# avi22bhattacharya/ThinkDiff-mlre

Hardware: AMD Instinct MI355X
Metric: images/sec (1024², 28 steps) ThinkDiff-CLIP FLUX.1 at 1/2/4/8 MI355X (higher is better)
Workload: dtype bf16

## Files before the change

### thinkdiff-mlre_amd/csrc/attention_bf16.hip

```cpp
#include "attention_common.h"

template <bool Q8>
__device__ __forceinline__ void attn_store_item(const TdAttnParams& p, const f32x16_t (&o)[4], const float inv, bf16_t* Ob, const int Sq,
                                                const int head, const int q, const int h5) {
  if constexpr (Q8) {
    if (p.q8) {
      const int qr = min(q, Sq - 1);
      attn_store_rows_q8(o, inv, p.q8 + (size_t)qr * p.ldq8 + head * D, h5, p.q8_inv[qr], p.q8_amax + qr, q < Sq);
      return;
    }
  }
  attn_store_rows(o, inv, Ob + (size_t)min(q, Sq - 1) * p.ldo + head * D, h5, (p.ldo & 7) == 0 && !(p.variant & 0x200), q < Sq);
}

template <bool CAUSAL, int NWAVES, bool BIAS = false, bool VARLEN = false, bool PRE = false, bool RS = true, bool FIXED = false, bool KVSEG = false>
__global__ __launch_bounds__(NWAVES * 64, 2) void td_attn_fwd_d128_lean_kernel(const TdAttnParams p) {
#if defined(__HIP_DEVICE_COMPILE__)
  extern __shared__ __attribute__((aligned(16))) char smem[];

  const int tid = threadIdx.x;
  const int lane = tid & 63;
  const int wid = __builtin_amdgcn_readfirstlane(tid >> 6);
  const int h5 = lane >> 5;
  const int l31 = lane & 31;

  const int qblk = blockIdx.x;
  const int head = blockIdx.y;
  const int batch = blockIdx.z;
  const int kvhead = head / p.q_per_kv;
  const int q0 = qblk * (NWAVES * Q_WAVE) + wid * Q_WAVE;

  const bf16_t* Qb = p.Q + (size_t)batch * p.q_bstride;
  const bf16_t* Kb = p.K + (size_t)batch * p.kv_bstride;
  const bf16_t* Vb = p.V + (size_t)batch * p.kv_bstride;
  bf16_t* Ob = p.O + (size_t)batch * p.o_bstride;
  int Sq = p.Sq, Skv = p.Skv, c_off = p.causal_offset;
  if constexpr (VARLEN) {
    const int r0 = p.seg_starts[batch];
    Sq = Skv = p.seg_starts[batch + 1] - r0;
    if (qblk * (NWAVES * Q_WAVE) >= Sq) return;
    if constexpr (KVSEG) {
      const int k0 = max(p.kv_seg_row0[batch], 0);
      Skv = max(p.kv_seg_lens[batch], Sq);
      c_off = Skv - Sq;
      Qb += (size_t)r0 * p.ldq; Kb += (size_t)k0 * p.ldkv; Vb += (size_t)k0 * p.ldkv; Ob += (size_t)r0 * p.ldo;
    } else {
      Qb += (size_t)r0 * p.ldq; Kb += (size_t)r0 * p.ldkv; Vb += (size_t)r0 * p.ldkv; Ob += (size_t)r0 * p.ldo;
    }
  }

  const unsigned q_bytes = (unsigned)(((long long)(Sq - 1) * p.ldq + p.Hq * D) * 2);
  if constexpr (CAUSAL) {
    if (p.kv_lens) { Skv = p.kv_lens[batch]; c_off = Skv - p.Sq; }
  }
  const unsigned kv_bytes = (unsigned)(((long long)(Skv - 1) * p.ldkv + p.Hkv * D) * 2);
  __amdgpu_buffer_rsrc_t rsQ = __builtin_amdgcn_make_buffer_rsrc((void*)Qb, 0, q_bytes, 0x00020000);
  __amdgpu_buffer_rsrc_t rsK = __builtin_amdgcn_make_buffer_rsrc((void*)Kb, 0, kv_bytes, 0x00020000);
  __amdgpu_buffer_rsrc_t rsV = __builtin_amdgcn_make_buffer_rsrc((void*)Vb, 0, kv_bytes, 0x00020000);

  int nt = (Skv + KV_TILE - 1) / KV_TILE;
  if (CAUSAL) {
    const int last_q = min(Sq, (qblk + 1) * NWAVES * Q_WAVE) - 1 + c_off;
    nt = min(nt, last_q / KV_TILE + 1);
  }

  constexpr int GROUPS = KV_TILE / 4;
  constexpr int SG = (GROUPS + NWAVES - 1) / NWAVES;
  const int srow = lane >> 4;
  unsigned voffK[SG];
#pragma unroll
  for (int s = 0; s < SG; ++s) {
    const int g = wid + NWAVES * s;
    const int swz = (srow << 2) | (g & 3);
    const int chunk = (lane & 15) ^ swz;
    voffK[s] = (unsigned)(g * 4 + srow) * (unsigned)p.ldkv * 2u + (unsigned)(kvhead * D + chunk * 8) * 2u;
  }
  auto stage = [&](int slot, int t) {
    const unsigned tile_off = (unsigned)t * KV_TILE * (unsigned)p.ldkv * 2u;
#pragma unroll
    for (int s = 0; s < SG; ++s) {
      const int g = wid + NWAVES * s;
      if (GROUPS % NWAVES == 0 || g < GROUPS) {
        __builtin_amdgcn_raw_ptr_buffer_load_lds(rsK, (TD_LDS void*)(smem + slot * TILE_BYTES + g * 1024), 16, voffK[s] + tile_off, 0, 0, 0);
        __builtin_amdgcn_raw_ptr_buffer_load_lds(rsV, (TD_LDS void*)(smem + (2 + slot) * TILE_BYTES + g * 1024), 16, voffK[s] + tile_off, 0, 0, 0);
      }
    }
  };
  stage(0, 0);

  bf16x8_t qf[8];
  {
    const unsigned qoff = (unsigned)(q0 + l31) * (unsigned)p.ldq * 2u + (unsigned)(head * D + 8 * h5) * 2u;
#pragma unroll
    for (int ks = 0; ks < 8; ++ks) {
      u32x4_t v = __builtin_amdgcn_raw_buffer_load_b128(rsQ, qoff + ks * 32, 0, 0);
      qf[ks] = __builtin_bit_cast(bf16x8_t, v);
    }
  }

  const unsigned lds0 = (unsigned)(uintptr_t)(TD_LDS char*)smem;
  unsigned ka[8];
  {
    const unsigned ksw = ((lane & 3) << 2) | ((lane >> 2) & 3);
#pragma unroll
    for (int ks = 0; ks < 8; ++ks) ka[ks] = lds0 + l31 * 256 + (((2 * ks + h5) ^ ksw) << 4);
  }
  unsigned va[2][4];
  {
    const unsigned vq = (lane & 15) >> 2, vp = lane & 3;
    const unsigned vchunk = 2 * ((lane >> 4) & 1) + (vp >> 1);
#pragma unroll
    for (int jj = 0; jj < 2; ++jj) {
      const unsigned swz = (vq << 2) | ((2 * jj + h5) & 3);
#pragma unroll
      for (int db = 0; db < 4; ++db)
        va[jj][db] = lds0 + 2 * TILE_BYTES + (4 * h5 + vq + 8 * jj) * 256 + (((4 * db + vchunk) ^ swz) << 4) + 8 * (vp & 1);
    }
  }

  f32x16_t o[4];
#pragma unroll
// ... 36 lines not shown
            for (int r = 0; r < 4; ++r) st[kb][4 * g4 + r] += bv[r] * inv_scale;
          }
        }
    }
    const bool need_mask = (key0 + KV_TILE > Skv) || (CAUSAL && key0 + KV_TILE - 1 > q0 + c_off);
    if (need_mask) {
#pragma unroll
      for (int kb = 0; kb < 2; ++kb)
#pragma unroll
        for (int r = 0; r < 16; ++r) {
          const int key = key0 + kb * 32 + (r & 3) + 8 * (r >> 2) + 4 * h5;
          if ((key >= Skv) || (CAUSAL && key > q_pos)) st[kb][r] = -INFINITY;
        }
    }

    attn_tile_softmax_pv<PO, PRE, RS, FIXED>(st, o, lacc, m_run, qnegm, t == 0, c, va, h5);
  };
  {
    int t = 0;
    for (; t + 1 < nt; t += 2) {
      tile(t, std::integral_constant<unsigned, 0>{});
      tile(t + 1, std::integral_constant<unsigned, 1>{});
    }
    if (t < nt) tile(t, std::integral_constant<unsigned, 0>{});
  }

  const float inv = 1.0f / (RS ? lacc[0] : half_swap_sum(lacc[0]));
  attn_store_item<!CAUSAL && !BIAS && !VARLEN>(p, o, inv, Ob, Sq, head, q0 + l31, h5);
#endif
}



template <int NWAVES, bool XCD_REMAP, bool PRE = false, bool RS = true, bool FIXED = false>
__global__ __launch_bounds__(NWAVES * 64, 2) void td_attn_fwd_d128_streamk_kernel(const TdAttnParams p, char* __restrict__ ws,
                                                                                  const int n_qblk, const int nt) {
#if defined(__HIP_DEVICE_COMPILE__)
  extern __shared__ __attribute__((aligned(16))) char smem[];
  const int tid = threadIdx.x;
  const int lane = tid & 63;
  const int wid = __builtin_amdgcn_readfirstlane(tid >> 6);
  const int h5 = lane >> 5;
  const int l31 = lane & 31;
  TD_LDS unsigned* const ticket_lds = (TD_LDS unsigned*)(smem + 4 * TILE_BYTES);

  const int G = gridDim.x;
  long long it, it_end;
  const int r = attn_sk_range<XCD_REMAP>((long long)n_qblk * p.Hq * p.batch * nt, it, it_end);

  const int Skv = p.Skv;
  constexpr int GROUPS = KV_TILE / 4;
  constexpr int SG = (GROUPS + NWAVES - 1) / NWAVES;
  const int srow = lane >> 4;
  const float c = p.scale * 1.4426950408889634f;
  const float cc = PRE ? 1.0f : c;
  const bf16x8_t kone = {(short)(h5 == 0 ? 0x3F80 : 0), 0, 0, 0, 0, 0, 0, 0};

  const unsigned lds0 = (unsigned)(uintptr_t)(TD_LDS char*)smem;
  unsigned ka[8];
  {
    const unsigned ksw = ((lane & 3) << 2) | ((lane >> 2) & 3);
#pragma unroll
    for (int ks = 0; ks < 8; ++ks) ka[ks] = lds0 + l31 * 256 + (((2 * ks + h5) ^ ksw) << 4);
  }
  unsigned va[2][4];
  {
    const unsigned vq = (lane & 15) >> 2, vp = lane & 3;
    const unsigned vchunk = 2 * ((lane >> 4) & 1) + (vp >> 1);
#pragma unroll
    for (int jj = 0; jj < 2; ++jj) {
      const unsigned swz = (vq << 2) | ((2 * jj + h5) & 3);
#pragma unroll
      for (int db = 0; db < 4; ++db)
        va[jj][db] = lds0 + 2 * TILE_BYTES + (4 * h5 + vq + 8 * jj) * 256 + (((4 * db + vchunk) ^ swz) << 4) + 8 * (vp & 1);
    }
  }

  if ((p.variant & 0x100) && wid >= 4) __builtin_amdgcn_s_setprio(1);
  while (it < it_end) {
    const int item = (int)(it / nt);
    const int kb = (int)(it - (long long)item * nt);
    const int ke = (int)min((long long)nt, kb + (it_end - it));
    __builtin_assume(ke > kb);
    it += ke - kb;
    const int qblk = item % n_qblk;
    const int hb = item / n_qblk;
    const int head = hb % p.Hq, batch = hb / p.Hq;
    const int kvhead = head / p.q_per_kv;
    const int q0 = qblk * (NWAVES * Q_WAVE) + wid * Q_WAVE;

    const bf16_t* Qb = p.Q + (size_t)batch * p.q_bstride;
    const bf16_t* Kb = p.K + (size_t)batch * p.kv_bstride;
    const bf16_t* Vb = p.V + (size_t)batch * p.kv_bstride;
    const unsigned q_bytes = (unsigned)(((long long)(p.Sq - 1) * p.ldq + p.Hq * D) * 2);
    const unsigned kv_bytes = (unsigned)(((long long)(Skv - 1) * p.ldkv + p.Hkv * D) * 2);
    __amdgpu_buffer_rsrc_t rsQ = __builtin_amdgcn_make_buffer_rsrc((void*)Qb, 0, q_bytes, 0x00020000);
    __amdgpu_buffer_rsrc_t rsK = __builtin_amdgcn_make_buffer_rsrc((void*)Kb, 0, kv_bytes, 0x00020000);
    __amdgpu_buffer_rsrc_t rsV = __builtin_amdgcn_make_buffer_rsrc((void*)Vb, 0, kv_bytes, 0x00020000);

    unsigned voffK[SG];
#pragma unroll
    for (int s = 0; s < SG; ++s) {
      const int g = wid + NWAVES * s;
      const int swz = (srow << 2) | (g & 3);
      const int chunk = (lane & 15) ^ swz;
      voffK[s] = (unsigned)(g * 4 + srow) * (unsigned)p.ldkv * 2u + (unsigned)(kvhead * D + chunk * 8) * 2u;
    }
    auto stage = [&](int slot, int t) {
      const unsigned tile_off = (unsigned)t * KV_TILE * (unsigned)p.ldkv * 2u;
#pragma unroll
      for (int s = 0; s < SG; ++s) {
        const int g = wid + NWAVES * s;
        if (GROUPS % NWAVES == 0 || g < GROUPS) {
          __builtin_amdgcn_raw_ptr_buffer_load_lds(rsK, (TD_LDS void*)(smem + slot * TILE_BYTES + g * 1024), 16, voffK[s] + tile_off, 0, 0, 0);
          __builtin_amdgcn_raw_ptr_buffer_load_lds(rsV, (TD_LDS void*)(smem + (2 + slot) * TILE_BYTES + g * 1024), 16, voffK[s] + tile_off, 0, 0, 0);
        }
      }
    };
    __syncthreads();
    stage(0, kb);

    bf16x8_t qf[8];
    {
      const unsigned qoff = (unsigned)(q0 + l31) * (unsigned)p.ldq * 2u + (unsigned)(head * D + 8 * h5) * 2u;
#pragma unroll
      for (int ks = 0; ks < 8; ++ks) {
        u32x4_t v = __builtin_amdgcn_raw_buffer_load_b128(rsQ, qoff + ks * 32, 0, 0);
        qf[ks] = __builtin_bit_cast(bf16x8_t, v);
      }
    }

    f32x16_t o[4];
#pragma unroll
    for (int db = 0; db < 4; ++db)
#pragma unroll
      for (int rr = 0; rr < 16; ++rr) o[db][rr] = 0.f;
    f32x16_t lacc;
#pragma unroll
    for (int rr = 0; rr < 16; ++rr) lacc[rr] = 0.f;
    float m_run = 0.f;
    bf16x8_t qnegm = {0, 0, 0, 0, 0, 0, 0, 0};
    auto tile = [&](const int t, auto slot_tag) {
      constexpr unsigned SLOT = decltype(slot_tag)::value;
      constexpr unsigned PO = SLOT * TILE_BYTES;
      asm volatile("s_waitcnt vmcnt(0)" ::: "memory");
      __syncthreads();
      if (t + 1 < ke) stage(SLOT ^ 1, t + 1);

      f32x16_t st[2];
      attn_tile_scores<PO, FIXED>(st, qf, kone, qnegm, ka);

      const int key0 = t * KV_TILE;
      if (key0 + KV_TILE > Skv) {
// ... 83 lines not shown
  }
  if (p.Sq == 1 && p.causal && !p.bias && !p.seg_starts && (p.variant & 0xff) == 0 && (p.kv_lens || p.causal_offset == p.Skv - 1))
    return td_attn_decode_launch(p, stream);
  TdAttnParams q = p;
  q.q_per_kv = p.Hq / p.Hkv;
  constexpr int NW = 8;
  constexpr int lds = 4 * TILE_BYTES;
  int dev = 0;
  TD_CHECK_HIP(hipGetDevice(&dev));
  dim3 grid((p.Sq + NW * Q_WAVE - 1) / (NW * Q_WAVE), p.Hq, p.batch);
  if (p.bias) TD_CHECK_ARG(p.Skv % 4 == 0 && ((uintptr_t)p.bias) % 16 == 0 && p.batch == 1, "td_attention: bias needs Skv %% 4 == 0, 16-byte alignment, batch 1");
  if (p.kv_lens) TD_CHECK_ARG(p.causal && !p.bias, "td_attention: per-sequence kv lengths exist for the causal kernel only");
  if (p.q_prescaled) TD_CHECK_ARG(!p.causal && !p.bias && !p.kv_lens && !p.seg_starts, "td_attention: pre-scaled q is a form of the joint (unmasked) attention only");
  TD_CHECK_ARG(p.score_bound >= 0.f && p.score_bound <= 48.f && (p.score_bound == 0.f || p.q_prescaled), "td_attention: a score bound goes with pre-scaled q (joint attention) and lies in (0, 48] octaves (0 = none)");
  if (p.q8) TD_CHECK_ARG(!p.causal && !p.bias && !p.kv_lens && !p.seg_starts && p.batch == 1 && p.q8_inv && p.q8_amax && p.ldq8 % 8 == 0 && ((uintptr_t)p.q8) % 8 == 0,
                         "td_attention: the int8 output form is for the joint attention of one batch entry, with 8-byte aligned rows");
  if (p.seg_starts && p.kv_seg_row0) {
    if (int e = attn_launch<td_attn_fwd_d128_lean_kernel<true, NW, false, true, false, true, false, true>>(grid, NW * 64, lds, stream, dev, q)) return e;
    TD_CHECK_LAUNCH();
    return 0;
  }
  if (p.seg_starts) {
    TD_CHECK_ARG(!p.bias && !p.kv_lens && p.Sq == p.Skv && (!p.causal || p.causal_offset == 0),
                 "td_attention(varlen): full or causal (offset 0) attention inside each segment only (no bias or cache lengths)");
    if (int e = p.causal ? attn_launch<td_attn_fwd_d128_lean_kernel<true, NW, false, true>>(grid, NW * 64, lds, stream, dev, q)
                         : attn_launch<td_attn_fwd_d128_lean_kernel<false, NW, false, true>>(grid, NW * 64, lds, stream, dev, q)) return e;
    TD_CHECK_LAUNCH();
    return 0;
  }

  const int n_items = (int)(grid.x * grid.y * grid.z);
  const int cus = device_cus(dev);
  const int nt = (p.Skv + KV_TILE - 1) / KV_TILE;
  int e;
  if (!p.causal && !p.bias && !p.kv_lens && (p.variant & 0xff) != 1 && cus > 0 && n_items > cus && cus < SK_MAX_RANGES && (long long)n_items * nt < (1ll << 31)) {
    char* ws = (char*)p.sk_ws;
    if (!ws) {
      if (int rc = sk_pooled_workspace(dev, cus, stream, &ws)) return rc;
    }
    constexpr int lds_sk = lds + 16;
    const dim3 ranges(cus);
    const int n_qblk = (int)grid.x;
    if (p.q_prescaled && p.score_bound > 0.f) e = attn_launch<td_attn_fwd_d128_streamk_kernel<NW, true, true, true, true>>(ranges, NW * 64, lds_sk, stream, dev, q, ws, n_qblk, nt);
    else if (p.q_prescaled) e = attn_launch<td_attn_fwd_d128_streamk_kernel<NW, true, true>>(ranges, NW * 64, lds_sk, stream, dev, q, ws, n_qblk, nt);
    else if ((p.variant & 0xff) == 2) e = attn_launch<td_attn_fwd_d128_streamk_kernel<NW, false>>(ranges, NW * 64, lds_sk, stream, dev, q, ws, n_qblk, nt);
    else e = attn_launch<td_attn_fwd_d128_streamk_kernel<NW, true>>(ranges, NW * 64, lds_sk, stream, dev, q, ws, n_qblk, nt);
  } else if (p.bias) {
    e = p.causal ? attn_launch<td_attn_fwd_d128_lean_kernel<true, NW, true>>(grid, NW * 64, lds, stream, dev, q)
                 : attn_launch<td_attn_fwd_d128_lean_kernel<false, NW, true>>(grid, NW * 64, lds, stream, dev, q);
  } else if (p.q_prescaled && p.score_bound > 0.f) {
    e = attn_launch<td_attn_fwd_d128_lean_kernel<false, NW, false, false, true, true, true>>(grid, NW * 64, lds, stream, dev, q);
  } else if (p.q_prescaled) {
    e = attn_launch<td_attn_fwd_d128_lean_kernel<false, NW, false, false, true>>(grid, NW * 64, lds, stream, dev, q);
  } else {
    e = p.causal ? attn_launch<td_attn_fwd_d128_lean_kernel<true, NW>>(grid, NW * 64, lds, stream, dev, q)
                 : attn_launch<td_attn_fwd_d128_lean_kernel<false, NW>>(grid, NW * 64, lds, stream, dev, q);
  }
  if (e) return e;
  TD_CHECK_LAUNCH();
  return 0;
}

size_t td_attn_streamk_ws_bytes() {
  int dev = 0;
  if (hipGetDevice(&dev) != hipSuccess) return 0;
  const int cus = device_cus(dev);
  return cus > 0 && cus < SK_MAX_RANGES ? sk_ws_bytes(cus) : 0;
}
```

### thinkdiff-mlre_amd/csrc/attention_common.h

```cpp
#pragma once
#include <atomic>
#include <mutex>
#include <type_traits>
#include <vector>

#include "td_common.h"
#include "td_kernels.h"

namespace {

constexpr int D = 128;
constexpr int KV_TILE = 64;
constexpr int Q_WAVE = 32;
constexpr int TILE_BYTES = KV_TILE * D * 2;

__device__ __forceinline__ void half_swap(float x, float& lo, float& hi) {
  lo = x;
  hi = x;
  asm volatile("s_nop 1\n\tv_permlane32_swap_b32 %0, %1\n\ts_nop 1" : "+v"(lo), "+v"(hi));
}
__device__ __forceinline__ float max3(float a, float b, float c) {
  float r;
  asm("v_max3_f32 %0, %1, %2, %3" : "=v"(r) : "v"(a), "v"(b), "v"(c));
  return r;
// ... 154 lines not shown
        w[0] = pack_bf2(o[db][4 * g] * inv, o[db][4 * g + 1] * inv);
        w[1] = pack_bf2(o[db][4 * g + 2] * inv, o[db][4 * g + 3] * inv);
        if (live) *(u32x2_t*)(row_ptr + 4 * h5 + db * 32 + 8 * g) = w;
      }
  }
}

__device__ __forceinline__ void attn_store_rows_q8(const f32x16_t (&o)[4], const float inv, uint8_t* row_ptr, const int h5, const float qinv, unsigned* amax,
                                                   const bool live) {
  float am = 0.f;
#pragma unroll
  for (int db = 0; db < 4; ++db)
#pragma unroll
    for (int g = 0; g < 4; g += 2) {
      unsigned w[2];
#pragma unroll
      for (int h = 0; h < 2; ++h) {
        unsigned acc = 0;
#pragma unroll
        for (int b = 0; b < 4; ++b) {
          const float v = rbf(o[db][4 * (g + h) + b] * inv);
          am = fmaxf(am, fabsf(v));
          acc |= ((unsigned)__float2int_rn(fminf(fmaxf(v * qinv, -127.f), 127.f)) & 0xffu) << (8 * b);
        }
        w[h] = acc;
      }
      const auto r = __builtin_amdgcn_permlane32_swap(w[0], w[1], false, false);
      if (live) *(u32x2_t*)(row_ptr + db * 32 + 8 * (g + h5)) = u32x2_t{r[0], r[1]};
    }
  am = half_swap_max(am);
  if (live && h5 == 0) __hip_atomic_fetch_max(amax, as_u32(am), __ATOMIC_RELAXED, __HIP_MEMORY_SCOPE_AGENT);
}

constexpr int SK_SLOT_FLOATS = 8 * 64 * 68;
constexpr int SK_HEADER_BYTES = 4096;
constexpr int SK_MAX_RANGES = SK_HEADER_BYTES / 4 - 16;

template <bool XCD_REMAP>
__device__ __forceinline__ int attn_sk_range(const long long total, long long& it, long long& it_end) {
  const int G = gridDim.x;
  int r = blockIdx.x;
  if constexpr (XCD_REMAP) {
    const int q8 = G >> 3, r8 = G & 7, xcd = r & 7;
    r = (xcd < r8 ? xcd * (q8 + 1) : r8 * (q8 + 1) + (xcd - r8) * q8) + (r >> 3);
  }
  it = total * r / G;
  it_end = total * (r + 1) / G;
  return r;
}

__device__ __forceinline__ bool attn_sk_handoff(f32x16_t (&o_io)[4], const float m_run, float& l_run, const float cc, const int r, const int G,
                                                const bool tail, char* ws, TD_LDS unsigned* const ticket_lds, const int tid, const int wid) {
  const int lane = tid & 63;
  f32x16_t o[4] = {o_io[0], o_io[1], o_io[2], o_io[3]};
  unsigned* const cnt = (unsigned*)ws + 16;
  const int j = tail ? r : r + 1;
  const __amdgpu_buffer_rsrc_t rsS = __builtin_amdgcn_make_buffer_rsrc((void*)(ws + SK_HEADER_BYTES), 0, (unsigned)(2 * G) * SK_SLOT_FLOATS * 4u, 0x00020000);
  const unsigned lane_off = ((unsigned)wid * 17u * 64u + (unsigned)lane) * 16u;
  const unsigned mine = (unsigned)(tail ? j : G + j) * (SK_SLOT_FLOATS * 4u) + lane_off;
  const unsigned theirs = (unsigned)(tail ? G + j : j) * (SK_SLOT_FLOATS * 4u) + lane_off;
  auto ask = [&](bool draw) -> unsigned {
    __syncthreads();
    if (tid == 0)
      *ticket_lds = draw ? __hip_atomic_fetch_add(cnt + j, 1u, __ATOMIC_RELAXED, __HIP_MEMORY_SCOPE_AGENT)
                         : __hip_atomic_load(cnt + j, __ATOMIC_RELAXED, __HIP_MEMORY_SCOPE_AGENT);
    __syncthreads();
    return *ticket_lds;
  };
  bool other_ready = !tail && ask(false) == 1u;
  if (!other_ready) {
#pragma unroll
    for (int q4 = 0; q4 < 16; ++q4) {
      const u32x4_t v = {as_u32(o[q4 >> 2][4 * (q4 & 3)]), as_u32(o[q4 >> 2][4 * (q4 & 3) + 1]),
                         as_u32(o[q4 >> 2][4 * (q4 & 3) + 2]), as_u32(o[q4 >> 2][4 * (q4 & 3) + 3])};
      __builtin_amdgcn_raw_buffer_store_b128(v, rsS, mine + q4 * 1024u, 0, 16);
    }
    const u32x4_t ml = {as_u32(m_run), as_u32(l_run), 0u, 0u};
    __builtin_amdgcn_raw_buffer_store_b128(ml, rsS, mine + 16 * 1024u, 0, 16);
    asm volatile("s_waitcnt vmcnt(0)" ::: "memory");
    other_ready = ask(true) == 1u;
    if (!other_ready) return false;
  }
  if (tid == 0) __builtin_amdgcn_fence(__ATOMIC_ACQUIRE, "agent");
  asm volatile("s_waitcnt vmcnt(0)" ::: "memory");
  __syncthreads();
  const u32x4_t ml = __builtin_amdgcn_raw_buffer_load_b128(rsS, theirs + 16 * 1024u, 0, 0);
  const float m2 = as_f32(ml[0]), l2 = as_f32(ml[1]);
  const float mm = fmaxf(m_run, m2);
  const float a1 = __builtin_amdgcn_exp2f((m_run - mm) * cc), a2 = __builtin_amdgcn_exp2f((m2 - mm) * cc);
  auto comb = [&](float own, float other) {
    return tail ? __builtin_fmaf(other, a2, own * a1) : __builtin_fmaf(own, a1, other * a2);
  };
  l_run = comb(l_run, l2);
#pragma unroll
  for (int q4 = 0; q4 < 16; ++q4) {
    const u32x4_t v = __builtin_amdgcn_raw_buffer_load_b128(rsS, theirs + q4 * 1024u, 0, 0);
#pragma unroll
    for (int k4 = 0; k4 < 4; ++k4)
      o[q4 >> 2][4 * (q4 & 3) + k4] = comb(o[q4 >> 2][4 * (q4 & 3) + k4], as_f32(v[k4]));
  }
  if (tid == 0) __hip_atomic_store(cnt + j, 0u, __ATOMIC_RELAXED, __HIP_MEMORY_SCOPE_AGENT);
#pragma unroll
  for (int db = 0; db < 4; ++db) o_io[db] = o[db];
  return true;
}

template <auto KERNEL, typename... Args>
int attn_launch(const dim3 grid, const int threads, const int lds, hipStream_t stream, const int dev, Args... args) {
  static std::atomic<unsigned long long> done{0};
  if (!((done.load(std::memory_order_acquire) >> (dev & 63)) & 1ull)) {
    TD_CHECK_HIP(hipFuncSetAttribute((const void*)KERNEL, hipFuncAttributeMaxDynamicSharedMemorySize, lds));
    done.fetch_or(1ull << (dev & 63), std::memory_order_release);
  }
  hipLaunchKernelGGL(KERNEL, grid, dim3(threads), lds, stream, args...);
  return 0;
}

}
```

### thinkdiff-mlre_amd/csrc/capi.hip

```cpp
#include <cstdarg>
#include <cstdio>
#include <initializer_list>
#include "td_kernels.h"
#include "../../include/thinkdiff_hip.h"

static thread_local char g_err[512] = "";

void td_set_error(const char* fmt, ...) {
  va_list ap;
  va_start(ap, fmt);
  vsnprintf(g_err, sizeof(g_err), fmt, ap);
  va_end(ap);
}

extern "C" {

const char* td_last_error(void) { return g_err; }
int td_abi_version(void) { return 24; }

int td_linear_bf16(const void* x, int64_t ldx, const void* w, const void* bias, void* y, int64_t ldy,
                   int M, int N, int K, int act, const void* gate, const void* res, int64_t ldr,
                   void* stream) {
  TdGemmParams p;
  p.A = (const bf16_t*)x; p.lda = (int)ldx;
// ... 78 lines not shown
int td_linear_f32out_bf16(const void* x, int64_t ldx, const void* w, const void* bias, float* y, int64_t ldy,
                          int M, int N, int K, void* stream) {
  TdGemmParams p;
  p.A = (const bf16_t*)x; p.lda = (int)ldx; p.W = (const bf16_t*)w; p.bias = (const bf16_t*)bias;
  p.C = (bf16_t*)y; p.ldc = (int)ldy; p.M = M; p.N = N; p.K = K; p.out_f32 = 1; p.cfg = (N <= 64) ? 1 : (M <= 32 ? 2 : 0);
  return td_gemm_launch(p, (hipStream_t)stream);
}

static int g_attn_variant = 0;
int td_attention_set_variant(int variant) {
  const int prev = g_attn_variant;
  g_attn_variant = variant;
  return prev;
}

int td_attention_bf16(const void* q, int64_t ldq, int64_t q_bstride, const void* k, const void* v,
                      int64_t ldkv, int64_t kv_bstride, void* o, int64_t ldo, int64_t o_bstride,
                      int batch, int Sq, int Skv, int Hq, int Hkv, int head_dim, float scale,
                      int causal, void* stream) {
  TdAttnParams p;
  p.Q = (const bf16_t*)q; p.K = (const bf16_t*)k; p.V = (const bf16_t*)v; p.O = (bf16_t*)o;
  p.batch = batch; p.Sq = Sq; p.Skv = Skv; p.Hq = Hq; p.Hkv = Hkv; p.head_dim = head_dim;
  p.ldq = (int)ldq; p.ldkv = (int)ldkv; p.ldo = (int)ldo;
  p.q_bstride = q_bstride; p.kv_bstride = kv_bstride; p.o_bstride = o_bstride;
  p.scale = scale; p.causal = causal; p.causal_offset = Skv - Sq; p.variant = g_attn_variant & ~0x800;
  p.q_prescaled = (g_attn_variant & 0x800) && !causal ? 1 : 0;
  return td_attn_launch(p, (hipStream_t)stream);
}

int td_attention_joint_prescaled_bf16(const void* q, int64_t ldq, const void* k, const void* v, int64_t ldkv, void* o, int64_t ldo, int S, int H, float score_bound, void* stream) {
  TdAttnParams p;
  p.Q = (const bf16_t*)q; p.K = (const bf16_t*)k; p.V = (const bf16_t*)v; p.O = (bf16_t*)o;
  p.batch = 1; p.Sq = S; p.Skv = S; p.Hq = H; p.Hkv = H; p.head_dim = 128;
  p.ldq = (int)ldq; p.ldkv = (int)ldkv; p.ldo = (int)ldo; p.scale = 1.0f; p.causal = 0; p.causal_offset = 0; p.variant = g_attn_variant & 0xff;
  p.q_prescaled = 1; p.score_bound = score_bound;
  return td_attn_launch(p, (hipStream_t)stream);
}

size_t td_attention_fp8_workspace_bytes(int Sq, int Skv, int Hq) { return Sq > 0 && Skv > 0 && Hq > 0 ? td_attn_fp8_ws_bytes(Sq, Skv, Hq) : 0; }

int td_attention_fp8(const void* q, int64_t ldq, const void* k, const void* v, int64_t ldkv, void* o, int64_t ldo,
                     int Sq, int Skv, int Hq, float scale, void* workspace, void* stream) {
  TdAttnParams p;
  p.Q = (const bf16_t*)q; p.K = (const bf16_t*)k; p.V = (const bf16_t*)v; p.O = (bf16_t*)o;
  p.batch = 1; p.Sq = Sq; p.Skv = Skv; p.Hq = Hq; p.Hkv = Hq; p.head_dim = 128;
  p.ldq = (int)ldq; p.ldkv = (int)ldkv; p.ldo = (int)ldo; p.scale = scale; p.f8_ws = workspace; p.variant = ((g_attn_variant & 1) ? 0x1000 : 0) | ((g_attn_variant & 2) ? 0x2000 : 0) | (((g_attn_variant >> 4) & 7) << 16);
  return td_attn_fp8_launch(p, (hipStream_t)stream);
}

int td_attention_fp8_qk_rope(const void* qkv, int64_t ld, int q_col, int k_col, int v_col, void* o, int64_t ldo, int S, int H,
                             const float* cos, const float* sin, int split, const void* wqA, const void* wkA, const void* wqB, const void* wkB,
                             float eps, float scale, void* workspace, void* stream) {
  TD_CHECK_ARG(qkv && cos && sin && q_col >= 0 && k_col >= 0 && v_col >= 0 && (q_col | k_col | v_col) % 8 == 0, "td_attention_fp8_qk_rope: projection buffer, both tables, 16-byte aligned column offsets");
  TD_CHECK_ARG(S > 0 && H > 0 && (long long)(q_col > k_col ? (q_col > v_col ? q_col : v_col) : (k_col > v_col ? k_col : v_col)) + (long long)H * 128 <= ld,
               "td_attention_fp8_qk_rope: the q / k / v head blocks (H=%d x 128 columns from their offsets) do not fit a row of ld=%lld", H, (long long)ld);
  TdAttnParams p;
  p.Q = (const bf16_t*)qkv + q_col; p.K = (const bf16_t*)qkv + k_col; p.V = (const bf16_t*)qkv + v_col; p.O = (bf16_t*)o;
  p.batch = 1; p.Sq = S; p.Skv = S; p.Hq = H; p.Hkv = H; p.head_dim = 128;
  p.ldq = (int)ld; p.ldkv = (int)ld; p.ldo = (int)ldo; p.scale = scale; p.f8_ws = workspace; p.variant = ((g_attn_variant & 1) ? 0x1000 : 0) | ((g_attn_variant & 2) ? 0x2000 : 0);
  p.rope_cos = cos; p.rope_sin = sin; p.rope_split = split; p.rope_eps = eps;
  p.rope_wqA = (const bf16_t*)wqA; p.rope_wkA = (const bf16_t*)wkA; p.rope_wqB = (const bf16_t*)wqB; p.rope_wkB = (const bf16_t*)wkB;
  return td_attn_fp8_launch(p, (hipStream_t)stream);
}

int td_attention_varlen_bf16(const void* q, int64_t ldq, const void* k, const void* v, int64_t ldkv, void* o, int64_t ldo,
                             const int* seg_starts, int n_seg, int max_len, int Hq, int Hkv, float scale, void* stream) {
  TD_CHECK_ARG(seg_starts && n_seg > 0 && max_len > 0, "td_attention_varlen: empty segment list");
// ... 650 lines not shown
```

### thinkdiff-mlre_amd/csrc/flux_engine.hip

```cpp
#include <cmath>
#include <cstring>
#include <functional>

#include "flux_model.h"

namespace {

struct TraceScope {
  td_flux* f; hipStream_t s; bool on;
  TraceScope(td_flux* f_, hipStream_t s_, int cat, double flops) : f(f_), s(s_), on(f_->tracing) {
    if (!on) return;
    const size_t i = f->trace.size();
    if (2 * i + 1 >= f->ev_pool.size()) { on = false; return; }
    f->trace.push_back({cat, flops});
    (void)hipEventRecord(f->ev_pool[2 * i], s);
  }
  ~TraceScope() {
    if (on) (void)hipEventRecord(f->ev_pool[2 * (f->trace.size() - 1) + 1], s);
  }
};

int gemm_p(td_flux* f, hipStream_t s, TdGemmParams p) {
  p.no_tail = f->shared_chip;
  const int rows = p.M + p.g_M;
// ... 95 lines not shown
}

int norm_rows(td_flux* f, hipStream_t s, const TdNormParams& p) {
  TraceScope ts(f, s, TD_TRACE_NORM, 0.0);
  return td_norm_rows_launch(p, s);
}
int qk_rope(td_flux* f, hipStream_t s, const TdQkRopeParams& p) {
  TraceScope ts(f, s, TD_TRACE_QKROPE, 0.0);
  return td_qk_norm_rope_launch(p, s);
}
int attn(td_flux* f, hipStream_t s, const TdAttnParams& p, const TdQkRopeParams* rope = nullptr, const int* ref_in = nullptr, int* ref_out = nullptr) {
  TraceScope ts(f, s, TD_TRACE_ATTN, 4.0 * p.Sq * (double)p.Skv * p.Hq * 128.0);
  if (f->m->attn_mode == TD_ATTENTION_FP8) {
    TdAttnParams q = p;
    q.f8_ws = f->attn8_ws;
    q.variant = p.variant & 0x1000;
    q.ref_in = ref_in; q.ref_out = ref_out;
    if (rope) {
      const TdQkRopeParams& r = *rope;
      q.rope_cos = r.cos; q.rope_sin = r.sin; q.rope_split = r.split; q.rope_eps = r.eps; q.rope_q_premul = r.q_premul;
      q.rope_wqA = r.wqA; q.rope_wkA = r.wkA; q.rope_wqB = r.wqB; q.rope_wkB = r.wkB;
    }
    return td_attn_fp8_launch(q, s);
  }
  return td_attn_launch(p, s);
}

struct Switches {
  int attn_tune;
  bool attn8_no_fuse;
  bool attn8_no_href;
  bool attn_no_bound;
  static Switches read() {
    static const int tune = getenv("TD_ATTN_TUNE") ? (int)strtol(getenv("TD_ATTN_TUNE"), nullptr, 0) & ~0xff : 0;
    return {tune, getenv("TD_ATTN8_NO_FUSE") != nullptr, getenv("TD_ATTN8_NO_HREF") != nullptr, getenv("TD_ATTN_NO_BOUND") != nullptr};
  }
};

int alloc_workspace(td_flux* f) {
  const FluxModel* m = f->m;
  const TdFluxConfig* cfg = &m->cfg;
  const int64_t D = m->D, M = m->M;
  const int max_img_tokens = m->max_img, max_txt_tokens = m->max_txt + (m->num_mode > 0 ? 1 : 0);
  const int64_t S = (int64_t)max_img_tokens + max_txt_tokens;
  const int64_t n = m->max_steps;
  struct Req { void** p; int64_t bytes; };
  std::vector<Req> reqs = {
      {(void**)&f->h, S * D * 2}, {(void**)&f->xn, S * D * 2}, {(void**)&f->qkv, S * 3 * D * 2},
      {(void**)&f->attn, S * D * 2}, {(void**)&f->mlp, S * M * 2}, {(void**)&f->cat, S * (D + M) * 2},
      {(void**)&f->ctx, (int64_t)max_txt_tokens * D * 2}, {(void**)&f->vout, (int64_t)max_img_tokens * m->Cout * 2},
      {(void**)&f->xin, m->Ccond > 0 ? (int64_t)max_img_tokens * m->Cin * 2 : 0},
      {(void**)&f->xref, m->Ccond == 0 ? (int64_t)max_img_tokens * m->Cout * 2 : 0},
      {(void**)&f->cn_E, m->controlnet ? (int64_t)max_img_tokens * D * 2 : 0},
      {(void**)&f->cn_samples, m->controlnet ? (int64_t)(cfg->num_layers + cfg->num_single_layers) * max_img_tokens * D * 2 : 0},
      {(void**)&f->tproj, n * 256 * 2}, {(void**)&f->tmid, n * D * 2}, {(void**)&f->te, n * D * 2},
      {(void**)&f->gproj, 256 * 2}, {(void**)&f->gmid, (int64_t)D * 2}, {(void**)&f->ge, (int64_t)D * 2},
      {(void**)&f->pmid, (int64_t)D * 2}, {(void**)&f->pe, (int64_t)D * 2},
      {(void**)&f->temb, n * D * 2}, {(void**)&f->st, n * D * 2}, {(void**)&f->mods, n * (int64_t)m->NMOD * 2},
      {(void**)&f->cosT, S * 128 * 4}, {(void**)&f->sinT, S * 128 * 4}, {(void**)&f->ids, S * 3 * 4},
      {(void**)&f->tvals, (n + 1) * 4},
      {(void**)&f->xq, S * (D + SM_EXT)}, {(void**)&f->aq, S * (D + M)}, {(void**)&f->xs, S * 4}, {(void**)&f->as_, S * 4},
      {(void**)&f->attn_ws, (int64_t)td_attn_streamk_ws_bytes()},
      {(void**)&f->attn8_ws, (int64_t)td_attn_fp8_ws_bytes((int)S, (int)S, cfg->num_heads)},
      {(void**)&f->href[0], (int64_t)(cfg->num_layers + cfg->num_single_layers) * cfg->num_heads * S * 4},
      {(void**)&f->href[1], (int64_t)(cfg->num_layers + cfg->num_single_layers) * cfg->num_heads * S * 4},
      {(void**)&f->hs_scale, (int64_t)(2 * cfg->num_layers + cfg->num_single_layers) * S * 4}, {(void**)&f->hs_inv, (int64_t)(2 * cfg->num_layers + cfg->num_single_layers) * S * 4},
      {(void**)&f->hs_amax, (int64_t)(2 * cfg->num_layers + cfg->num_single_layers) * S * 4},
// ... 949 lines not shown
```

Before: 0.6250.

## Add 16x16x32 MFMA attention body for score-bound prescaled bf16 attention

Adds an alternate attention inner loop for the prescaled, score-bound, non-causal path. It uses 16x16x32 bf16 MFMA instead of the 32x32 form, with a new V staging swizzle and new LDS address maps. Row sums come from an MFMA against a ones vector, and the stream-K handoff gains a plain-sum merge mode. Both the lean and stream-K kernels dispatch to it by default unless FP8 output is requested or a force-32 variant bit is set. This aims at better MFMA throughput and register use in the exp/PV stage, at the cost of a second code path with its own layout and precision behaviour.

```diff
diff --git a/thinkdiff-mlre_amd/csrc/attention_bf16.hip b/thinkdiff-mlre_amd/csrc/attention_bf16.hip
--- a/thinkdiff-mlre_amd/csrc/attention_bf16.hip
+++ b/thinkdiff-mlre_amd/csrc/attention_bf16.hip
@@ -13,7 +13,7 @@
   attn_store_rows(o, inv, Ob + (size_t)min(q, Sq - 1) * p.ldo + head * D, h5, (p.ldo & 7) == 0 && !(p.variant & 0x200), q < Sq);
 }
 
-template <bool CAUSAL, int NWAVES, bool BIAS = false, bool VARLEN = false, bool PRE = false, bool RS = true, bool FIXED = false, bool KVSEG = false>
+template <bool CAUSAL, int NWAVES, bool BIAS = false, bool VARLEN = false, bool PRE = false, bool RS = true, bool FIXED = false, bool KVSEG = false, bool M16 = false>
 __global__ __launch_bounds__(NWAVES * 64, 2) void td_attn_fwd_d128_lean_kernel(const TdAttnParams p) {
 #if defined(__HIP_DEVICE_COMPILE__)
   extern __shared__ __attribute__((aligned(16))) char smem[];
@@ -67,13 +67,14 @@
   constexpr int GROUPS = KV_TILE / 4;
   constexpr int SG = (GROUPS + NWAVES - 1) / NWAVES;
   const int srow = lane >> 4;
-  unsigned voffK[SG];
+  unsigned voffK[SG], voffV[SG];
 #pragma unroll
   for (int s = 0; s < SG; ++s) {
     const int g = wid + NWAVES * s;
     const int swz = (srow << 2) | (g & 3);
     const int chunk = (lane & 15) ^ swz;
     voffK[s] = (unsigned)(g * 4 + srow) * (unsigned)p.ldkv * 2u + (unsigned)(kvhead * D + chunk * 8) * 2u;
+    voffV[s] = M16 ? (unsigned)(g * 4 + srow) * (unsigned)p.ldkv * 2u + (unsigned)(kvhead * D + attn16_v_src_chunk(g, lane) * 8) * 2u : voffK[s];
   }
   auto stage = [&](int slot, int t) {
     const unsigned tile_off = (unsigned)t * KV_TILE * (unsigned)p.ldkv * 2u;
@@ -82,11 +83,30 @@
       const int g = wid + NWAVES * s;
       if (GROUPS % NWAVES == 0 || g < GROUPS) {
         __builtin_amdgcn_raw_ptr_buffer_load_lds(rsK, (TD_LDS void*)(smem + slot * TILE_BYTES + g * 1024), 16, voffK[s] + tile_off, 0, 0, 0);
-        __builtin_amdgcn_raw_ptr_buffer_load_lds(rsV, (TD_LDS void*)(smem + (2 + slot) * TILE_BYTES + g * 1024), 16, voffK[s] + tile_off, 0, 0, 0);
+        __builtin_amdgcn_raw_ptr_buffer_load_lds(rsV, (TD_LDS void*)(smem + (2 + slot) * TILE_BYTES + g * 1024), 16, voffV[s] + tile_off, 0, 0, 0);
       }
     }
   };
   stage(0, 0);
+
+  if constexpr (M16) {
+    static_assert(!CAUSAL && !BIAS && !VARLEN && PRE && RS && FIXED, "the 16x16x32 body serves the score-bound joint form only");
+    bf16x8_t qf[2][4];
+    attn16_load_q(qf, rsQ, q0, head, p.ldq, lane);
+    unsigned ka[4], va[8];
+    attn16_lds_addrs((unsigned)(uintptr_t)(TD_LDS char*)smem, lane, ka, va);
+    f32x4_t o[8][2], ls[2];
+#pragma unroll
+    for (int i = 0; i < 4; ++i) {
+#pragma unroll
+      for (int dt = 0; dt < 8; ++dt) o[dt][0][i] = o[dt][1][i] = 0.f;
+      ls[0][i] = ls[1][i] = 0.f;
+    }
+    attn16_run_tiles(o, ls, qf, ka, va, 0, nt, Skv, lane, stage);
+    const float l[2] = {ls[0][0], ls[1][0]};
+    attn16_store_rows(o, l, Ob + head * D, p.ldo, q0, Sq, lane, (p.ldo & 7) == 0 && !(p.variant & 0x200));
+    return;
+  }
 
   bf16x8_t qf[8];
   {
@@ -189,7 +209,7 @@
 
 
 
-template <int NWAVES, bool XCD_REMAP, bool PRE = false, bool RS = true, bool FIXED = false>
+template <int NWAVES, bool XCD_REMAP, bool PRE = false, bool RS = true, bool FIXED = false, bool M16 = false>
 __global__ __launch_bounds__(NWAVES * 64, 2) void td_attn_fwd_d128_streamk_kernel(const TdAttnParams p, char* __restrict__ ws,
                                                                                   const int n_qblk, const int nt) {
 #if defined(__HIP_DEVICE_COMPILE__)
@@ -232,6 +252,9 @@
         va[jj][db] = lds0 + 2 * TILE_BYTES + (4 * h5 + vq + 8 * jj) * 256 + (((4 * db + vchunk) ^ swz) << 4) + 8 * (vp & 1);
     }
   }
+
+  unsigned ka16[4], va16[8];
+  if constexpr (M16) attn16_lds_addrs(lds0, lane, ka16, va16);
 
   if ((p.variant & 0x100) && wid >= 4) __builtin_amdgcn_s_setprio(1);
   while (it < it_end) {
@@ -255,13 +278,14 @@
     __amdgpu_buffer_rsrc_t rsK = __builtin_amdgcn_make_buffer_rsrc((void*)Kb, 0, kv_bytes, 0x00020000);
     __amdgpu_buffer_rsrc_t rsV = __builtin_amdgcn_make_buffer_rsrc((void*)Vb, 0, kv_bytes, 0x00020000);
 
-    unsigned voffK[SG];
+    unsigned voffK[SG], voffV[SG];
 #pragma unroll
     for (int s = 0; s < SG; ++s) {
       const int g = wid + NWAVES * s;
       const int swz = (srow << 2) | (g & 3);
       const int chunk = (lane & 15) ^ swz;
       voffK[s] = (unsigned)(g * 4 + srow) * (unsigned)p.ldkv * 2u + (unsigned)(kvhead * D + chunk * 8) * 2u;
+      voffV[s] = M16 ? (unsigned)(g * 4 + srow) * (unsigned)p.ldkv * 2u + (unsigned)(kvhead * D + attn16_v_src_chunk(g, lane) * 8) * 2u : voffK[s];
     }
     auto stage = [&](int slot, int t) {
       const unsigned tile_off = (unsigned)t * KV_TILE * (unsigned)p.ldkv * 2u;
@@ -270,12 +294,37 @@
         const int g = wid + NWAVES * s;
         if (GROUPS % NWAVES == 0 || g < GROUPS) {
           __builtin_amdgcn_raw_ptr_buffer_load_lds(rsK, (TD_LDS void*)(smem + slot * TILE_BYTES + g * 1024), 16, voffK[s] + tile_off, 0, 0, 0);
-          __builtin_amdgcn_raw_ptr_buffer_load_lds(rsV, (TD_LDS void*)(smem + (2 + slot) * TILE_BYTES + g * 1024), 16, voffK[s] + tile_off, 0, 0, 0);
+          __builtin_amdgcn_raw_ptr_buffer_load_lds(rsV, (TD_LDS void*)(smem + (2 + slot) * TILE_BYTES + g * 1024), 16, voffV[s] + tile_off, 0, 0, 0);
         }
       }
     };
     __syncthreads();
     stage(0, kb);
+
+    if constexpr (M16) {
+      static_assert(PRE && RS && FIXED, "the 16x16x32 body serves the score-bound form only");
+      bf16x8_t qf[2][4];
+      attn16_load_q(qf, rsQ, q0, head, p.ldq, lane);
+      f32x4_t o[8][2], ls[2];
+#pragma unroll
+      for (int i = 0; i < 4; ++i) {
+#pragma unroll
+        for (int dt = 0; dt < 8; ++dt) o[dt][0][i] = o[dt][1][i] = 0.f;
+        ls[0][i] = ls[1][i] = 0.f;
+      }
+      attn16_run_tiles(o, ls, qf, ka16, va16, kb, ke, Skv, lane, stage);
+      float l[2] = {ls[0][0], ls[1][0]};
+      if (kb > 0 || ke < nt) {
+        f32x16_t o16[4];
+#pragma unroll
+        for (int n = 0; n < 64; ++n) o16[n >> 4][n & 15] = o[n >> 3][(n >> 2) & 1][n & 3];
+        if (!attn_sk_handoff<true>(o16, l[1], l[0], 1.0f, r, G, kb > 0, ws, ticket_lds, tid, wid)) continue;
+#pragma unroll
+        for (int n = 0; n < 64; ++n) o[n >> 3][(n >> 2) & 1][n & 3] = o16[n >> 4][n & 15];
+      }
+      attn16_store_rows(o, l, p.O + (size_t)batch * p.o_bstride + head * D, p.ldo, q0, p.Sq, lane, (p.ldo & 7) == 0 && !(p.variant & 0x200));
+      continue;
+    }
 
     bf16x8_t qf[8];
     {
@@ -425,6 +474,7 @@
   const int n_items = (int)(grid.x * grid.y * grid.z);
   const int cus = device_cus(dev);
   const int nt = (p.Skv + KV_TILE - 1) / KV_TILE;
+  const bool m16 = !p.q8 && !(p.variant & M16_FORCE_32);
   int e;
   if (!p.causal && !p.bias && !p.kv_lens && (p.variant & 0xff) != 1 && cus > 0 && n_items > cus && cus < SK_MAX_RANGES && (long long)n_items * nt < (1ll << 31)) {
     char* ws = (char*)p.sk_ws;
@@ -434,13 +484,16 @@
     constexpr int lds_sk = lds + 16;
     const dim3 ranges(cus);
     const int n_qblk = (int)grid.x;
-    if (p.q_prescaled && p.score_bound > 0.f) e = attn_launch<td_attn_fwd_d128_streamk_kernel<NW, true, true, true, true>>(ranges, NW * 64, lds_sk, stream, dev, q, ws, n_qblk, nt);
+    if (p.q_prescaled && p.score_bound > 0.f && m16) e = attn_launch<td_attn_fwd_d128_streamk_kernel<NW, true, true, true, true, true>>(ranges, NW * 64, lds_sk, stream, dev, q, ws, n_qblk, nt);
+    else if (p.q_prescaled && p.score_bound > 0.f) e = attn_launch<td_attn_fwd_d128_streamk_kernel<NW, true, true, true, true>>(ranges, NW * 64, lds_sk, stream, dev, q, ws, n_qblk, nt);
     else if (p.q_prescaled) e = attn_launch<td_attn_fwd_d128_streamk_kernel<NW, true, true>>(ranges, NW * 64, lds_sk, stream, dev, q, ws, n_qblk, nt);
     else if ((p.variant & 0xff) == 2) e = attn_launch<td_attn_fwd_d128_streamk_kernel<NW, false>>(ranges, NW * 64, lds_sk, stream, dev, q, ws, n_qblk, nt);
     else e = attn_launch<td_attn_fwd_d128_streamk_kernel<NW, true>>(ranges, NW * 64, lds_sk, stream, dev, q, ws, n_qblk, nt);
   } else if (p.bias) {
     e = p.causal ? attn_launch<td_attn_fwd_d128_lean_kernel<true, NW, true>>(grid, NW * 64, lds, stream, dev, q)
                  : attn_launch<td_attn_fwd_d128_lean_kernel<false, NW, true>>(grid, NW * 64, lds, stream, dev, q);
+  } else if (p.q_prescaled && p.score_bound > 0.f && m16) {
+    e = attn_launch<td_attn_fwd_d128_lean_kernel<false, NW, false, false, true, true, true, false, true>>(grid, NW * 64, lds, stream, dev, q);
   } else if (p.q_prescaled && p.score_bound > 0.f) {
     e = attn_launch<td_attn_fwd_d128_lean_kernel<false, NW, false, false, true, true, true>>(grid, NW * 64, lds, stream, dev, q);
   } else if (p.q_prescaled) {
diff --git a/thinkdiff-mlre_amd/csrc/attention_common.h b/thinkdiff-mlre_amd/csrc/attention_common.h
--- a/thinkdiff-mlre_amd/csrc/attention_common.h
+++ b/thinkdiff-mlre_amd/csrc/attention_common.h
@@ -210,6 +210,146 @@
   if (live && h5 == 0) __hip_atomic_fetch_max(amax, as_u32(am), __ATOMIC_RELAXED, __HIP_MEMORY_SCOPE_AGENT);
 }
 
+constexpr int M16_FORCE_32 = 0x400;
+
+__device__ __forceinline__ int attn16_v_src_chunk(const int grp, const int lane) { return (lane & 15) ^ (((grp & 3) << 2) | (lane >> 4)); }
+
+__device__ __forceinline__ void attn16_lds_addrs(const unsigned lds0, const int lane, unsigned (&ka)[4], unsigned (&va)[8]) {
+  const unsigned i16 = lane & 15, g = lane >> 4;
+  const unsigned ksw = ((i16 & 3) << 2) | (i16 >> 2);
+#pragma unroll
+  for (int ks = 0; ks < 4; ++ks) ka[ks] = lds0 + i16 * 256 + (((4 * g + ks) ^ ksw) << 4);
+  const unsigned vq = i16 >> 2, pb = i16 & 3;
+#pragma unroll
+  for (int dt = 0; dt < 8; ++dt)
+    va[dt] = lds0 + 2 * TILE_BYTES + (4 * g + vq) * 256 + ((((pb ^ g) << 2) | ((dt >> 1) ^ vq)) << 4) + 8 * ((dt ^ pb) & 1);
+}
+
+__device__ __forceinline__ void attn16_load_q(bf16x8_t (&qf)[2][4], const __amdgpu_buffer_rsrc_t rsQ, const int q0, const int head, const int ldq, const int lane) {
+  const unsigned qoff = (unsigned)(q0 + (lane & 15)) * (unsigned)ldq * 2u + (unsigned)(head * D + 32 * (lane >> 4)) * 2u;
+#pragma unroll
+  for (int qb = 0; qb < 2; ++qb)
+#pragma unroll
+    for (int ks = 0; ks < 4; ++ks)
+      qf[qb][ks] = __builtin_bit_cast(bf16x8_t, __builtin_amdgcn_raw_buffer_load_b128(rsQ, qoff + (unsigned)qb * 16u * (unsigned)ldq * 2u + ks * 16, 0, 0));
+}
+
+template <unsigned PO>
+__device__ __forceinline__ void attn16_tile_scores(f32x4_t (&st)[4][2], const bf16x8_t (&qf)[2][4], const unsigned (&ka)[4]) {
+  constexpr int KPF = 2;
+  const f32x4_t zero4 = {0.f, 0.f, 0.f, 0.f};
+  auto kread = [&](int e) {
+    return *(const TD_LDS bf16x8_t*)(uintptr_t)(ka[e >> 2] + PO + (e & 3) * 16 * 256);
+  };
+  bf16x8_t kf[16];
+#pragma unroll
+  for (int e = 0; e < KPF; ++e) kf[e] = kread(e);
+  __builtin_amdgcn_sched_group_barrier(0x100, KPF, 0);
+#pragma unroll
+  for (int e = 0; e < 16; ++e) {
+    if (e + KPF < 16) kf[e + KPF] = kread(e + KPF);
+#pragma unroll
+    for (int qb = 0; qb < 2; ++qb)
+      st[e & 3][qb] = __builtin_amdgcn_mfma_f32_16x16x32_bf16(kf[e], qf[qb][e >> 2], e < 4 ? zero4 : st[e & 3][qb], 0, 0, 0);
+    if (e + KPF < 16) __builtin_amdgcn_sched_group_barrier(0x100, 1, 0);
+    __builtin_amdgcn_sched_group_barrier(0x008, 2, 0);
+  }
+}
+
+template <unsigned PO>
+__device__ __forceinline__ void attn16_tile_softmax_pv(const f32x4_t (&st)[4][2], f32x4_t (&o)[8][2], f32x4_t (&ls)[2], const unsigned (&va)[8]) {
+  bf16x8_t pf[2][2];
+#pragma unroll
+  for (int u = 0; u < 2; ++u)
+#pragma unroll
+    for (int qb = 0; qb < 2; ++qb) {
+      u32x4_t pk;
+#pragma unroll
+      for (int h = 0; h < 2; ++h) {
+        const f32x4_t s = st[2 * u + h][qb];
+        pk[2 * h] = pack_bf2(__builtin_amdgcn_exp2f(s[0]), __builtin_amdgcn_exp2f(s[1]));
+        pk[2 * h + 1] = pack_bf2(__builtin_amdgcn_exp2f(s[2]), __builtin_amdgcn_exp2f(s[3]));
+      }
+      pf[u][qb] = __builtin_bit_cast(bf16x8_t, pk);
+    }
+  constexpr int VPF = 2;
+  const bf16x8_t ones8 = {0x3F80, 0x3F80, 0x3F80, 0x3F80, 0x3F80, 0x3F80, 0x3F80, 0x3F80};
+  bf16x4_t v0[16], v1[16];
+  attn_static_for<VPF>([&](auto ec) {
+    constexpr int e = decltype(ec)::value;
+    v0[e] = attn_ds_read_tr16<PO + (e >> 3) * 32 * 256>(va[e & 7]);
+    v1[e] = attn_ds_read_tr16<PO + (e >> 3) * 32 * 256 + 16 * 256>(va[e & 7]);
+  });
+  attn_static_for<16>([&](auto ec) {
+    constexpr int e = decltype(ec)::value;
+    if constexpr (e + VPF < 16) {
+      v0[e + VPF] = attn_ds_read_tr16<PO + ((e + VPF) >> 3) * 32 * 256>(va[(e + VPF) & 7]);
+      v1[e + VPF] = attn_ds_read_tr16<PO + ((e + VPF) >> 3) * 32 * 256 + 16 * 256>(va[(e + VPF) & 7]);
+    }
+    constexpr int behind = 2 * (15 - e < VPF ? 15 - e : VPF);
+    asm volatile("s_waitcnt lgkmcnt(%2)" : "+v"(v0[e]), "+v"(v1[e]) : "n"(behind));
+    const bf16x8_t vf = __builtin_shufflevector(v0[e], v1[e], 0, 1, 2, 3, 4, 5, 6, 7);
+    o[e & 7][0] = __builtin_amdgcn_mfma_f32_16x16x32_bf16(vf, pf[e >> 3][0], o[e & 7][0], 0, 0, 0);
+    o[e & 7][1] = __builtin_amdgcn_mfma_f32_16x16x32_bf16(vf, pf[e >> 3][1], o[e & 7][1], 0, 0, 0);
+    if constexpr ((e & 3) == 3) ls[(e >> 2) & 1] = __builtin_amdgcn_mfma_f32_16x16x32_bf16(ones8, pf[e >> 3][(e >> 2) & 1], ls[(e >> 2) & 1], 0, 0, 0);
+    __builtin_amdgcn_sched_barrier(0x006);
+  });
+}
+
+template <typename STAGE>
+__device__ __forceinline__ void attn16_run_tiles(f32x4_t (&o)[8][2], f32x4_t (&ls)[2], const bf16x8_t (&qf)[2][4], const unsigned (&ka)[4], const unsigned (&va)[8],
+                                                 const int kb, const int ke, const int Skv, const int lane, STAGE&& stage) {
+  auto tile = [&](const int t, auto slot_tag) {
+    constexpr unsigned SLOT = decltype(slot_tag)::value;
+    constexpr unsigned PO = SLOT * TILE_BYTES;
+    asm volatile("s_waitcnt vmcnt(0)" ::: "memory");
+    __syncthreads();
+    if (t + 1 < ke) stage(SLOT ^ 1, t + 1);
+    f32x4_t st[4][2];
+    attn16_tile_scores<PO>(st, qf, ka);
+    const int key0 = t * KV_TILE + 4 * (lane >> 4);
+    if (t * KV_TILE + KV_TILE > Skv) {
+#pragma unroll
+      for (int kk = 0; kk < 4; ++kk)
+#pragma unroll
+        for (int qb = 0; qb < 2; ++qb)
+#pragma unroll
+          for (int i = 0; i < 4; ++i)
+            if (key0 + 16 * kk + i >= Skv) st[kk][qb][i] = -INFINITY;
+    }
+    attn16_tile_softmax_pv<PO>(st, o, ls, va);
+  };
+  int t = kb;
+  for (; t + 1 < ke; t += 2) {
+    tile(t, std::integral_constant<unsigned, 0>{});
+    tile(t + 1, std::integral_constant<unsigned, 1>{});
+  }
+  if (t < ke) tile(t, std::integral_constant<unsigned, 0>{});
+}
+
+__device__ __forceinline__ void attn16_store_rows(const f32x4_t (&o)[8][2], const float (&l)[2], bf16_t* Oh, const int ldo, const int q0, const int Sq, const int lane,
+                                                  const bool wide) {
+  const int g = lane >> 4;
+  const bool odd = g & 1;
+#pragma unroll
+  for (int qb = 0; qb < 2; ++qb) {
+    const int q = q0 + 16 * qb + (lane & 15);
+    const float inv = 1.0f / l[qb];
+    bf16_t* const row_ptr = Oh + (size_t)min(q, Sq - 1) * ldo + 32 * g;
+#pragma unroll
+    for (int c = 0; c < 4; ++c) {
+      const f32x4_t a = o[2 * c][qb], b = o[2 * c + 1][qb];
+      const unsigned a0 = pack_bf2(a[0] * inv, a[1] * inv), a1 = pack_bf2(a[2] * inv, a[3] * inv);
+      const unsigned b0 = pack_bf2(b[0] * inv, b[1] * inv), b1 = pack_bf2(b[2] * inv, b[3] * inv);
+      const u32x4_t w = {odd ? b0 : a0, odd ? b1 : a1, odd ? a0 : b0, odd ? a1 : b1};
+      if (q < Sq) {
+        if (wide) *(u32x4_t*)(row_ptr + 8 * c) = w;
+        else { *(u32x2_t*)(row_ptr + 8 * c) = u32x2_t{w[0], w[1]}; *(u32x2_t*)(row_ptr + 8 * c + 4) = u32x2_t{w[2], w[3]}; }
+      }
+    }
+  }
+}
+
 constexpr int SK_SLOT_FLOATS = 8 * 64 * 68;
 constexpr int SK_HEADER_BYTES = 4096;
 constexpr int SK_MAX_RANGES = SK_HEADER_BYTES / 4 - 16;
@@ -227,7 +367,8 @@
   return r;
 }
 
-__device__ __forceinline__ bool attn_sk_handoff(f32x16_t (&o_io)[4], const float m_run, float& l_run, const float cc, const int r, const int G,
+template <bool SUMS2 = false>
+__device__ __forceinline__ bool attn_sk_handoff(f32x16_t (&o_io)[4], float& m_run, float& l_run, const float cc, const int r, const int G,
                                                 const bool tail, char* ws, TD_LDS unsigned* const ticket_lds, const int tid, const int wid) {
   const int lane = tid & 63;
   f32x16_t o[4] = {o_io[0], o_io[1], o_io[2], o_io[3]};
@@ -267,9 +408,11 @@
   const float mm = fmaxf(m_run, m2);
   const float a1 = __builtin_amdgcn_exp2f((m_run - mm) * cc), a2 = __builtin_amdgcn_exp2f((m2 - mm) * cc);
   auto comb = [&](float own, float other) {
+    if constexpr (SUMS2) return own + other;
     return tail ? __builtin_fmaf(other, a2, own * a1) : __builtin_fmaf(own, a1, other * a2);
   };
   l_run = comb(l_run, l2);
+  if constexpr (SUMS2) m_run = comb(m_run, m2);
 #pragma unroll
   for (int q4 = 0; q4 < 16; ++q4) {
     const u32x4_t v = __builtin_amdgcn_raw_buffer_load_b128(rsS, theirs + q4 * 1024u, 0, 0);
diff --git a/thinkdiff-mlre_amd/csrc/capi.hip b/thinkdiff-mlre_amd/csrc/capi.hip
--- a/thinkdiff-mlre_amd/csrc/capi.hip
+++ b/thinkdiff-mlre_amd/csrc/capi.hip
@@ -134,7 +134,7 @@
   TdAttnParams p;
   p.Q = (const bf16_t*)q; p.K = (const bf16_t*)k; p.V = (const bf16_t*)v; p.O = (bf16_t*)o;
   p.batch = 1; p.Sq = S; p.Skv = S; p.Hq = H; p.Hkv = H; p.head_dim = 128;
-  p.ldq = (int)ldq; p.ldkv = (int)ldkv; p.ldo = (int)ldo; p.scale = 1.0f; p.causal = 0; p.causal_offset = 0; p.variant = g_attn_variant & 0xff;
+  p.ldq = (int)ldq; p.ldkv = (int)ldkv; p.ldo = (int)ldo; p.scale = 1.0f; p.causal = 0; p.causal_offset = 0; p.variant = g_attn_variant & 0x4ff;
   p.q_prescaled = 1; p.score_bound = score_bound;
   return td_attn_launch(p, (hipStream_t)stream);
 }
diff --git a/thinkdiff-mlre_amd/csrc/flux_engine.hip b/thinkdiff-mlre_amd/csrc/flux_engine.hip
--- a/thinkdiff-mlre_amd/csrc/flux_engine.hip
+++ b/thinkdiff-mlre_amd/csrc/flux_engine.hip
@@ -151,7 +151,8 @@
   bool attn8_no_href;
   bool attn_no_bound;
   static Switches read() {
-    static const int tune = getenv("TD_ATTN_TUNE") ? (int)strtol(getenv("TD_ATTN_TUNE"), nullptr, 0) & ~0xff : 0;
+    const char* const at = getenv("TD_ATTN_TUNE");
+    const int tune = at ? (int)strtol(at, nullptr, 0) & ~0xff : 0;
     return {tune, getenv("TD_ATTN8_NO_FUSE") != nullptr, getenv("TD_ATTN8_NO_HREF") != nullptr, getenv("TD_ATTN_NO_BOUND") != nullptr};
   }
 };
```

New measurement: 0.6343 (median of 6 runs). 1.01x the previous value.
